# linhthi/BLISS-GNN

Measured on AMD Instinct MI355X. Metric: steps/sec (train step: sample_blocks + gather + SAGE fwd/bwd + Adam + exp3), reddit-like, higher is better.
Workload: dtype bf16

## Files before the change

### bliss_gnn_amd/csrc/sampler.hip

```cpp
#include "common.cuh"
#include "bliss_gnn.h"
#include "prof.h"
#include "edge_q.cuh"
#include <cstdlib>

#ifndef TPB
#define TPB 256
#endif
#define ITEMS 4
#define CHUNK (TPB * ITEMS)

namespace {

#define SPAN (64 * ITEMS)
#define SEG_ZERO_WGS 8
#define LONG_COL 1024
#define LONG_FIRST 4096

struct alignas(8) ColEnt {
  int k, n;
  long long p0;
};

struct EdgeAt {
// ... 522 lines not shown
        if (i < n) x[r] = wc[i];
      }
#pragma unroll
      for (int r = 0; r < COL_RB; ++r) wr.set(r, x[r]);
    }
#pragma unroll
    for (int r = 0; r < COL_RB; ++r)
      if (t + r * COL_TPB < n) emax = max(emax, bf_exp_field(wr.get(r)));
#pragma unroll 8
    for (int i = t + COL_RB * COL_TPB; i < n; i += COL_TPB) emax = max(emax, bf_exp_field(wc[i]));
    const int wfrac = rel_frac(FRAC_DST, block_max_u31<COL_TPB>(emax, sh));
    const PlainRange wr_ok = bf_plain_range(wfrac);
    bool odd = false;
#pragma unroll
    for (int r = 0; r < COL_RB; ++r)
      if (wave0 + r * COL_TPB < n) {
        odd |= t + r * COL_TPB < n && !bf_is_plain(wr.get(r), wr_ok);
        part += bf_fixed_plain(wr.get(r), wfrac);
      }
#pragma unroll 8
    for (int i = t + COL_RB * COL_TPB; i < n; i += COL_TPB) {
      const bf16_t b = wc[i];
      odd |= !bf_is_plain(b, wr_ok);
      part += bf_fixed_plain(b, wfrac);
    }
    long long lost;
    long long ws_fixed = block_sum2_i64<COL_TPB>(part, odd ? 1 : 0, sh2, &lost);
    bf16_t wsum;
    if (lost == 0) wsum = fixed_to_bf(ws_fixed, wfrac, &bad);
    else {
      long long part_lo = 0;
      int sticky = 0;
      part = 0;
#pragma unroll 4
      for (int i = t; i < n; i += COL_TPB) part += bf_to_fixed_wide(wc[i], wfrac, &part_lo, &sticky, &bad);
      ws_fixed = block_sum2_i64<COL_TPB>(part, (part_lo != 0 || sticky) ? 1 : 0, sh2, &lost);
      if (lost == 0) wsum = fixed_to_bf(ws_fixed, wfrac, &bad);
      else {
        const long long lo_tot = block_sum_i64<COL_TPB>(part_lo, sh);
        const long long st_tot = block_sum_i64<COL_TPB>(sticky, sh);
        wsum = fixed_wide_to_bf(ws_fixed, lo_tot, st_tot != 0, wfrac, &bad);
      }
    }
    const float a = rbf((1.0f / (float)n) * eta_f);
    const PlainRange q_ok = bf_plain_range(FRAC_DST);
    part = 0; odd = false;
#pragma unroll
    for (int r = 0; r < COL_RB; ++r)
      if (wave0 + r * COL_TPB < n) {
        const bool in = t + r * COL_TPB < n;
        const bf16_t q = edge_q_pre(wr.get(r), wsum, a, ome_f);
        odd |= in && !bf_is_plain(q, q_ok);
        part += in ? bf_fixed_plain(q, FRAC_DST) : 0ll;
      }
#pragma unroll 8
    for (int i = t + COL_RB * COL_TPB; i < n; i += COL_TPB) {
      const bf16_t q = edge_q_pre(wc[i], wsum, a, ome_f);
      odd |= !bf_is_plain(q, q_ok);
      part += bf_fixed_plain(q, FRAC_DST);
    }
    long long qs_fixed = block_sum2_i64<COL_TPB>(part, odd ? 1 : 0, sh2, &lost);
    if (lost != 0) {
      part = 0;
#pragma unroll 4
      for (int i = t; i < n; i += COL_TPB) part += bf_to_fixed(edge_q_pre(wc[i], wsum, a, ome_f), FRAC_DST, &bad);
      qs_fixed = block_sum_i64<COL_TPB>(part, sh);
    }
    if (t == 0) col_store(k, ws_fixed, qs_fixed, wsum, n, eta_f, acc_w, acc_q, seed_coef, &bad);
  }
  }
  if (bad) atomicOr(&cnt->err, bad);
}

template <bool BANDIT>
__global__ void __launch_bounds__(BIN_TPB) k_bin_scatter(const int64_t* __restrict__ indptr, const int* __restrict__ indices,
                                                     const bf16_t* __restrict__ w, const int* __restrict__ seeds,
                                                     const int* __restrict__ seg_ptr, const long long* __restrict__ col_base,
    const int* __restrict__ span_seg, LayerCounts* cnt,
                                                     const unsigned long long* __restrict__ acc_w,
                                                     const unsigned long long* __restrict__ acc_q, float eta_f, float ome_f,
                                                     int uniform_nodes, int n_bins, int log2_bins, long long bin_cap, int* bin_cursor,
                                                     unsigned long long* __restrict__ bin_rec, unsigned* __restrict__ bitmap,
                                                     const uint2* __restrict__ seed_coef) {
  __shared__ int hist[MAX_BINS];
  __shared__ int gbase[MAX_BINS];
  const int S = cnt->S, E = cnt->E, tid = threadIdx.x;
  const int nb = (E + BIN_BATCH - 1) / BIN_BATCH;
  const int bmask = n_bins - 1;
  int bad = 0;
  for (int batch = blockIdx.x; batch < nb; batch += gridDim.x) {
    for (int b = tid; b < n_bins; b += BIN_TPB) hist[b] = 0;
    if (tid < BIN_BATCH / 32) bitmap[batch * (BIN_BATCH / 32) + tid] = 0u;
    __syncthreads();
    int srcs[BIN_ITEMS], ranks[BIN_ITEMS];
    bf16_t ts[BIN_ITEMS];
    const int wbase = batch * BIN_BATCH + (tid >> 6) * (64 * BIN_ITEMS);
    int hint = span_seg[wbase >> 8];
#pragma unroll
    for (int j = 0; j < BIN_ITEMS; ++j) {
      ranks[j] = -1; srcs[j] = 0; ts[j] = 0;
      const int base = wbase + j * 64;
      if (base >= E) continue;
      EdgeAt a = decode(base, E, S, seg_ptr, col_base, indices, &hint);
      if (a.k >= 0) {
        bf16_t t;
        if (uniform_nodes) {
          t = (bf16_t)0x3f80;
        } else if (BANDIT) {
          const uint2 cf = seed_coef[a.k];
          bf16_t q = edge_q_pre(w[a.pos], (bf16_t)(cf.x & 0xffffu), __uint_as_float(cf.y), ome_f);
          float r = rbf(bf2f(q) / bf2f((bf16_t)(cf.x >> 16)));
          t = f2bf(r * r);
        } else {
          float x = bf2f(w[a.pos]);
          t = f2bf(x * x);
        }
        srcs[j] = a.src; ts[j] = t;
        ranks[j] = atomicAdd(&hist[a.src & bmask], 1);
      }
    }
    __syncthreads();
    for (int b = tid; b < n_bins; b += BIN_TPB) {
      const int h = hist[b];
      int g0 = 0;
      if (h) {
        g0 = atomicAdd(bin_cursor + b, h);
        if ((long long)g0 + h > bin_cap) bad |= BLISS_ERR_CAP_CAND;
      }
      gbase[b] = g0;
    }
    __syncthreads();
#pragma unroll
    for (int j = 0; j < BIN_ITEMS; ++j) {
      if (ranks[j] >= 0) {
        const int b = srcs[j] & bmask;
        const long long idx = (long long)gbase[b] + ranks[j];
        if (idx < bin_cap) {
          const size_t o = (size_t)b * (size_t)bin_cap + (size_t)idx;
          const unsigned e = (unsigned)(wbase + j * 64 + lane_id());
          bin_rec[o] = ((unsigned long long)e << 32) | ((unsigned long long)((unsigned)srcs[j] >> log2_bins) << 15) | (ts[j] & 0x7fffu);
        }
      }
    }
    __syncthreads();
  }
  if (bad) atomicOr(&cnt->err, bad);
}

__global__ void __launch_bounds__(BINRED_TPB) k_bin_reduce(LayerCounts* cnt, int n_bins, int log2_bins, long long bin_cap,
                                                           int* bin_cursor, const unsigned long long* __restrict__ bin_rec,
                                                           int num_nodes, int slots,
                                                           const int* __restrict__ local_id, unsigned long long* __restrict__ seed_p2,
                                                           unsigned long long* __restrict__ touched_key,
                                                           unsigned long long* __restrict__ touched_sum, unsigned* bitmap, int cap_c) {
  extern __shared__ unsigned long long dyn_lds[];
  unsigned long long* sm = dyn_lds;
  unsigned* mn = (unsigned*)(dyn_lds + slots);
  const int b = blockIdx.x, tid = threadIdx.x;
  if (cnt->E == 0) return;
  const int ne = b < num_nodes ? ((num_nodes - 1 - b) >> log2_bins) + 1 : 0;
  for (int i = tid; i < ne; i += BINRED_TPB) { sm[i] = 0ull; mn[i] = 0xffffffffu; }
  __syncthreads();
  long long n = bin_cursor[b];
  if (n > bin_cap) n = bin_cap;
  const unsigned long long* rec = bin_rec + (size_t)b * (size_t)bin_cap;
  int bad = 0;
  for (long long i = tid; i < n; i += BINRED_TPB) {
    const unsigned long long r = rec[i];
    const int li = (int)(((unsigned)r) >> 15);
    atomicMin(&mn[li], (unsigned)(r >> 32));
    const int64_t fx = bf_to_fixed((bf16_t)(r & 0x7fffu), FRAC_SRC, &bad);
    if (fx) atomicAdd(&sm[li], (unsigned long long)fx);
  }
  __syncthreads();
  __shared__ int wg_cnt, wg_base;
  if (tid == 0) wg_cnt = 0;
  __syncthreads();
  for (int li = tid; li < ne; li += BINRED_TPB) {
    bool is_cand = false;
    if (mn[li] != 0xffffffffu) {
      const int lid = local_id[((unsigned)li << log2_bins) | (unsigned)b];
      if (lid >= 0) { seed_p2[lid] = sm[li]; mn[li] = 0xffffffffu; }
      else is_cand = true;
    }
    const unsigned long long mask = __ballot(is_cand);
    if (mask && lane_id() == 0) atomicAdd(&wg_cnt, __popcll(mask));
  }
  __syncthreads();
  if (tid == 0) { wg_base = wg_cnt ? atomicAdd(bin_cursor + n_bins, wg_cnt) : 0; wg_cnt = 0; }
  __syncthreads();
  for (int li = tid; li < ne; li += BINRED_TPB) {
    const unsigned fp = mn[li];
    if (fp != 0xffffffffu) {
      const int j = wg_base + atomicAdd(&wg_cnt, 1);
      if (j < cap_c) { touched_key[j] = ((unsigned long long)fp << 32) | (((unsigned)li << log2_bins) | (unsigned)b); touched_sum[j] = sm[li]; }
      atomicOr(bitmap + (fp >> 5), 1u << (fp & 31u));
    }
  }
  if (bad) atomicOr(&cnt->err, bad);
}

#define BTILE_W 4
#define BTILE (1024 * BTILE_W)
#define MAX_TILES 2048
__global__ void __launch_bounds__(1024) k_bitmap_tiles(const unsigned* __restrict__ bitmap, int* __restrict__ word_prefix,
                                                       int* __restrict__ tile_sum, LayerCounts* cnt) {
  __shared__ int sh[17];
  const int nw = (cnt->E + 31) >> 5;
  const int ntiles = (nw + BTILE - 1) / BTILE;
  for (int tile = blockIdx.x; tile < ntiles; tile += gridDim.x) {
    const int i = tile * BTILE + threadIdx.x * BTILE_W;
    uint4 v = make_uint4(0, 0, 0, 0);
    if (i < nw) v = *reinterpret_cast<const uint4*>(bitmap + i);
    const int c0 = __popc(v.x), c1 = __popc(v.y), c2 = __popc(v.z), c3 = __popc(v.w);
    int total, ex = block_excl_scan(c0 + c1 + c2 + c3, sh, &total);
    if (i < nw) *reinterpret_cast<int4*>(word_prefix + i) = make_int4(ex, ex + c0, ex + c0 + c1, ex + c0 + c1 + c2);
    if (threadIdx.x == 0) tile_sum[tile] = total;
  }
}

__device__ __forceinline__ double block_sum_f64(double v, double* shd) {
  for (int d = 32; d >= 1; d >>= 1) {
    long long b = __double_as_longlong(v);
    int lo = __shfl_down((int)(b & 0xffffffffll), d), hi = __shfl_down((int)(b >> 32), d);
    v += __longlong_as_double(((long long)hi << 32) | (unsigned)lo);
  }
  __syncthreads();
  if (lane_id() == 0) shd[threadIdx.x >> 6] = v;
  __syncthreads();
  double t = 0;
  for (int i = 0; i < (int)(blockDim.x >> 6); ++i) t += shd[i];
  return t;
}

template <bool COHERENT>
__device__ __forceinline__ void poisson_scale_body(int* hist, LayerCounts* cnt, int C, int num, double eps, int* rng_ctl,
                                                   int* layer_off, int is_last, int rng_cap_total, int* __restrict__ sel_state,
                                                   double* shd) {
  for (int i = threadIdx.x; i < (C + CHUNK - 1) / CHUNK + 2; i += 1024) sel_state[i] = 0;
  if (rng_ctl && threadIdx.x == 1023) rng_stream_acquire(rng_ctl, C, layer_off, is_last, rng_cap_total);
  int n[HIST_BINS / 1024];
  bool any = false;
#pragma unroll
  for (int i = 0; i < HIST_BINS / 1024; ++i) {
    const int b = i * 1024 + threadIdx.x;
    n[i] = COHERENT ? __hip_atomic_load(hist + b, __ATOMIC_RELAXED, __HIP_MEMORY_SCOPE_AGENT) : hist[b];
  }
#pragma unroll
  for (int i = 0; i < HIST_BINS / 1024; ++i) {
    const int b = i * 1024 + threadIdx.x;
    if (n[i]) {
      if (COHERENT) __hip_atomic_store(hist + b, 0, __ATOMIC_RELAXED, __HIP_MEMORY_SCOPE_AGENT); else hist[b] = 0;
      any = true;
    }
  }
  if (C <= num) {
    if (threadIdx.x == 0) { cnt->c = 1.0; cnt->all_one = 1; cnt->iters = 0; }
    return;
  }
  double c = 1.0;
  int it = 0;
  for (; it < 50; ++it) {
    const float c32 = (float)c;
    double loc = 0;
    if (any) {
#pragma unroll
      for (int i = 0; i < HIST_BINS / 1024; ++i) {
        if (n[i]) {
          float v = rbf(bf2f((bf16_t)(i * 1024 + threadIdx.x)) * c32);
          v = v < 1.0f ? v : (v != v ? v : 1.0f);
          loc += (double)n[i] * (double)v;
        }
      }
    }
    double Ssum = block_sum_f64(loc, shd);
    double lo = Ssum < (double)num ? Ssum : (double)num, hi = Ssum < (double)num ? (double)num : Ssum;
    if (lo / hi >= eps) { ++it; break; }
    c *= (double)num / Ssum;
  }
  if (threadIdx.x == 0) { cnt->c = c; cnt->all_one = 0; cnt->iters = it > 50 ? 50 : it; }
}

__global__ void __launch_bounds__(1024) k_poisson_scale(int* hist, LayerCounts* cnt, int num, double eps, int* rng_ctl,
                                                        int* layer_off, int is_last, int rng_cap_total, int* __restrict__ sel_state) {
  __shared__ double shd[16];
  poisson_scale_body<false>(hist, cnt, cnt->C, num, eps, rng_ctl, layer_off, is_last, rng_cap_total, sel_state, shd);
}

struct FusedScale { int* ticket; int num; double eps; int* rng_ctl; int* layer_off; int is_last; int rng_cap_total; int* sel_state; };
__global__ void __launch_bounds__(FIN_TPB) k_cand_number(const int* __restrict__ seeds, LayerCounts* cnt, int* __restrict__ cand_nid,
                                                         int* local_id, const unsigned long long* __restrict__ seed_p2,
                                                         const unsigned long long* __restrict__ touched_key,
                                                         const unsigned long long* __restrict__ touched_sum,
                                                         const unsigned* __restrict__ bitmap, const int* __restrict__ word_prefix,
                                                         const int* __restrict__ tile_sum, bf16_t* __restrict__ p, int* hist,
                                                         int cap_c, int uniform_nodes, const FusedScale fs) {
  __shared__ int lh[HWIN_N + 4];
  __shared__ int tile_off[MAX_TILES];
  __shared__ int sh[17];
  const int S = cnt->S;
  const int ntiles = (((cnt->E + 31) >> 5) + BTILE - 1) / BTILE;
  int run = 0;
  for (int base = 0; base < ntiles; base += FIN_TPB) {
    const int t = base + threadIdx.x;
    int total, ex = block_excl_scan(t < ntiles ? tile_sum[t] : 0, sh, &total);
    if (t < ntiles) tile_off[t] = run + ex;
    run += total;
  }
  int C = S + run;
  if (C > cap_c) { C = cap_c; if (blockIdx.x == 0 && threadIdx.x == 0) atomicOr(&cnt->err, BLISS_ERR_CAP_CAND); }
  if (blockIdx.x == 0 && threadIdx.x == 0) cnt->C = C;
  if (blockIdx.x != 0 && (int)blockIdx.x * FIN_TPB >= C) return;
  {
    int4* lh4 = reinterpret_cast<int4*>(lh);
    for (int b = threadIdx.x; b < (HWIN_N + 4) / 4; b += FIN_TPB) lh4[b] = make_int4(0, 0, 0, 0);
  }
  __syncthreads();
  int bad = 0;
  for (int i = blockIdx.x * FIN_TPB + threadIdx.x; i < C; i += gridDim.x * FIN_TPB) {
    int id;
    unsigned long long raw;
    if (i < S) {
      id = i; raw = seed_p2[i];
      cand_nid[i] = seeds[i];
    } else {
      const unsigned long long key = touched_key[i - S];
      raw = touched_sum[i - S];
      const unsigned fp = (unsigned)(key >> 32), g = (unsigned)key;
      id = S + tile_off[(fp >> 5) / BTILE] + word_prefix[fp >> 5] + __popc(bitmap[fp >> 5] & ((1u << (fp & 31u)) - 1u));
      if (id >= cap_c) continue;
      local_id[g] = id; cand_nid[id] = (int)g;
    }
    bf16_t pj;
    if (uniform_nodes) pj = raw ? (bf16_t)0x3f80 : (bf16_t)0;
    else pj = f2bf(sqrtf(bf2f(fixed_to_bf((int64_t)raw, FRAC_SRC, &bad))));
    p[id] = pj;
    if (pj >= HIST_BINS) bad |= BLISS_ERR_NONFINITE;
    else if ((unsigned)(pj - HWIN_LO) < (unsigned)HWIN_N) atomicAdd(&lh[pj - HWIN_LO], 1);
    else if (pj == 0) atomicAdd(&lh[HWIN_N], 1);
    else atomicAdd(hist + pj, 1);
  }
  __syncthreads();
  {
    const int4* lh4 = reinterpret_cast<const int4*>(lh);
    for (int b = threadIdx.x; b < HWIN_N / 4; b += FIN_TPB) {
      const int4 v = lh4[b];
      if (v.x | v.y | v.z | v.w) {
        if (v.x) atomicAdd(hist + HWIN_LO + 4 * b, v.x);
        if (v.y) atomicAdd(hist + HWIN_LO + 4 * b + 1, v.y);
        if (v.z) atomicAdd(hist + HWIN_LO + 4 * b + 2, v.z);
        if (v.w) atomicAdd(hist + HWIN_LO + 4 * b + 3, v.w);
      }
    }
    if (threadIdx.x == 0 && lh[HWIN_N]) atomicAdd(hist, lh[HWIN_N]);
  }
  if (bad) atomicOr(&cnt->err, bad);
  if (fs.ticket) {
    static_assert(FIN_TPB == 1024, "the fused Poisson scale runs in a 1024-thread workgroup");
    __shared__ int sh_is_last;
    __shared__ double shd[16];
    int active = (C + FIN_TPB - 1) / FIN_TPB;
    if (active > (int)gridDim.x) active = (int)gridDim.x;
    if (active < 1) active = 1;
    asm volatile("s_waitcnt vmcnt(0)" ::: "memory");
    __syncthreads();
    if (threadIdx.x == 0) {
      sh_is_last = atomicAdd(fs.ticket, 1) == active - 1;
      if (sh_is_last) __hip_atomic_store(fs.ticket, 0, __ATOMIC_RELAXED, __HIP_MEMORY_SCOPE_AGENT);
    }
    __syncthreads();
    if (sh_is_last)
      poisson_scale_body<true>(hist, cnt, C, fs.num, fs.eps, fs.rng_ctl, fs.layer_off, fs.is_last, fs.rng_cap_total, fs.sel_state, shd);
  }
}

__device__ __forceinline__ bf16_t incl_prob(const bf16_t* __restrict__ p, int j, int S, int all_one, float c32) {
  if (all_one || j < S) return 0x3f80;
  float v = rbf(bf2f(p[j]) * c32);
  return (v < 1.0f || v != v) ? f2bf(v) : (bf16_t)0x3f80;
}

#define SEL_AGG 1
#define SEL_PFX 2
__global__ void __launch_bounds__(TPB) k_select_fused(const bf16_t* __restrict__ p, const float* __restrict__ uniforms_base,
                                                      const int* __restrict__ u_off, LayerCounts* cnt, bf16_t* __restrict__ P,
                                                      int* state, const int* __restrict__ cand_nid, int* __restrict__ new_id,
                                                      int* __restrict__ kept_nid, bf16_t* __restrict__ node_prob, int cap_c, int cap_k,
                                                      int* __restrict__ kept_map) {
  __shared__ int sh4[TPB / 64];
  __shared__ int sh_chunk, sh_base, sh_K;
  const float* __restrict__ uniforms = uniforms_base + (u_off ? *u_off : 0);
  const int S = cnt->S, C = min(cnt->C, cap_c), all_one = cnt->all_one;
  const float c32 = (float)cnt->c;
  const int nchunks = (C + CHUNK - 1) / CHUNK;
  if (threadIdx.x == 0) sh_chunk = atomicAdd(state, 1);
  __syncthreads();
  const int chunk = sh_chunk;
  if (chunk >= nchunks) return;
  unsigned long long mask[ITEMS];
  bf16_t Pv[ITEMS];
  int wave_total = 0;
#pragma unroll
  for (int i = 0; i < ITEMS; ++i) {
    const int j = chunk * CHUNK + (threadIdx.x >> 6) * SPAN + i * 64 + lane_id();
    bool keep = false;
    Pv[i] = 0;
    if (j < C) {
      Pv[i] = incl_prob(p, j, S, all_one, c32);
      P[j] = Pv[i];
      keep = __hip_atomic_load(uniforms + j, __ATOMIC_RELAXED, __HIP_MEMORY_SCOPE_AGENT) < bf2f(Pv[i]);
    }
    mask[i] = __ballot(keep);
    wave_total += __popcll(mask[i]);
  }
  int tot;
  const int woff = chunk_wave_offset(wave_total, sh4, &tot);
  if (threadIdx.x < 64) {
    const int lane = lane_id();
    int excl = 0, bad = 0;
    if (chunk > 0) {
      if (lane == 0) __hip_atomic_store(state + 1 + chunk, (tot << 2) | SEL_AGG, __ATOMIC_RELAXED, __HIP_MEMORY_SCOPE_AGENT);
      long long spins = 0;
      for (int top = chunk - 1; top >= 0;) {
        const int j = top - lane;
        const int v = j >= 0 ? __hip_atomic_load(state + 1 + j, __ATOMIC_RELAXED, __HIP_MEMORY_SCOPE_AGENT) : SEL_PFX;
        const unsigned long long ready = __ballot((v & 3) != 0), pfx = __ballot((v & 3) == SEL_PFX);
        const int stop = pfx ? __ffsll((long long)pfx) - 1 : 63;
        const unsigned long long need = stop == 63 ? ~0ull : ((1ull << (stop + 1)) - 1ull);
        if ((ready & need) != need) {
          __builtin_amdgcn_s_sleep(1);
          if (++spins > (1ll << 22)) { bad = BLISS_ERR_CAP_KEPT; break; }
          continue;
        }
        excl += wave_total_i32(lane <= stop && j >= 0 ? (v >> 2) : 0);
        if (pfx) break;
        top -= 64;
      }
    }
    if (lane == 0) {
      __hip_atomic_store(state + 1 + chunk, ((excl + tot) << 2) | SEL_PFX, __ATOMIC_RELAXED, __HIP_MEMORY_SCOPE_AGENT);
      sh_base = excl;
      if (chunk == nchunks - 1) {
        int K = excl + tot;
        if (K > cap_k) { bad |= BLISS_ERR_CAP_KEPT; K = cap_k; }
        cnt->K = K;
        sh_K = K;
      }
      if (bad) atomicOr(&cnt->err, bad);
    }
  }
  __syncthreads();
  int run = sh_base + woff;
#pragma unroll
  for (int i = 0; i < ITEMS; ++i) {
    const int j = chunk * CHUNK + (threadIdx.x >> 6) * SPAN + i * 64 + lane_id();
    if (j < C) {
      const bool keep = (mask[i] >> lane_id()) & 1ull;
      const int r = run + __popcll(mask[i] & ((1ull << lane_id()) - 1ull));
      if (keep && r < cap_k) {
        const int g = cand_nid[j];
        kept_nid[r] = g; node_prob[r] = Pv[i]; new_id[j] = r;
        if (kept_map) kept_map[g] = r;
      } else new_id[j] = -1;
    }
    run += __popcll(mask[i]);
  }
  if (chunk == nchunks - 1)
    for (int r = sh_K + threadIdx.x; r < cap_k; r += TPB) { kept_nid[r] = 0; node_prob[r] = 0x3f80; }
}

__global__ void __launch_bounds__(TPB) k_mn_prepare(LayerCounts* cnt, const bf16_t* __restrict__ p, bf16_t* __restrict__ P,
                                                    int* __restrict__ new_id, int cap_c) {
  const int C = min(cnt->C, cap_c);
  for (int j = blockIdx.x * TPB + threadIdx.x; j < C; j += gridDim.x * TPB) { P[j] = p[j]; new_id[j] = 0; }
}
__global__ void __launch_bounds__(TPB) k_mn_mark(LayerCounts* cnt, const int* __restrict__ chosen, int n_chosen, int* __restrict__ new_id, int cap_c) {
  const int C = min(cnt->C, cap_c);
  for (int i = blockIdx.x * TPB + threadIdx.x; i < n_chosen; i += gridDim.x * TPB) {
    const int j = chosen[i];
    if (j >= 0 && j < C) new_id[j] = 1; else atomicOr(&cnt->err, BLISS_ERR_CAP_CAND);
  }
}
__global__ void __launch_bounds__(TPB) k_mn_copy_p(const LayerCounts* cnt, const bf16_t* __restrict__ p, bf16_t* __restrict__ P, int cap_c) {
  const int C = min(cnt->C, cap_c);
  for (int j = blockIdx.x * TPB + threadIdx.x; j < C; j += gridDim.x * TPB) P[j] = p[j];
}
template <bool EMIT>
__global__ void __launch_bounds__(TPB) k_mn_select(LayerCounts* cnt, const bf16_t* __restrict__ P, int* __restrict__ chunk_io,
                                                   const int* __restrict__ cand_nid, int* __restrict__ new_id,
                                                   int* __restrict__ kept_nid, bf16_t* __restrict__ node_prob, int cap_c, int cap_k,
                                                   int* __restrict__ kept_map) {
  __shared__ int sh4[TPB / 64];
  const int S = cnt->S, C = min(cnt->C, cap_c);
  const int nchunks = (C + CHUNK - 1) / CHUNK;
  for (int chunk = blockIdx.x; chunk < nchunks; chunk += gridDim.x) {
    unsigned long long mask[ITEMS];
    int drawn[ITEMS];
    int wave_total = 0;
#pragma unroll
    for (int i = 0; i < ITEMS; ++i) {
      const int j = chunk * CHUNK + (threadIdx.x >> 6) * SPAN + i * 64 + lane_id();
      drawn[i] = j < C ? (EMIT ? new_id[j] : new_id[j] == 1) : 0;
      mask[i] = __ballot(j < C && (drawn[i] == 1 || j < S));
      wave_total += __popcll(mask[i]);
    }
    int tot;
    const int woff = chunk_wave_offset(wave_total, sh4, &tot);
    if (!EMIT) { if (threadIdx.x == 0) chunk_io[chunk] = tot; continue; }
    int run = chunk_io[chunk] + woff;
#pragma unroll
    for (int i = 0; i < ITEMS; ++i) {
      const int j = chunk * CHUNK + (threadIdx.x >> 6) * SPAN + i * 64 + lane_id();
      if (j < C) {
        const bool in_u = (mask[i] >> lane_id()) & 1ull;
        const int r = run + __popcll(mask[i] & ((1ull << lane_id()) - 1ull));
        if (in_u && r < cap_k) {
          const int g = cand_nid[j];
          kept_nid[r] = g; node_prob[r] = P[j]; new_id[j] = drawn[i] == 1 ? r : -2 - r;
          if (kept_map && drawn[i] == 1) kept_map[g] = r;
        } else new_id[j] = -1;
      }
      run += __popcll(mask[i]);
    }
  }
  if (EMIT) {
    const int K = min(cnt->K, cap_k);
// ... 200 lines not shown
}

#define TSORT_MAX_S 32768
__global__ void __launch_bounds__(TPB) k_tr_sort_lists(const int* __restrict__ t_indptr, const int* __restrict__ t_unsorted,
                                                       const int* __restrict__ dst, LayerCounts* cnt, int cap_k, int cap_s,
                                                       int* __restrict__ t_edge, const int* __restrict__ cand_nid, int* local_id,
                                                       int cap_c, const int* __restrict__ kept_nid, int* kept_map, int do_cleanup) {
  extern __shared__ unsigned bm_all[];
  if (do_cleanup) maps_cleanup(cnt, cand_nid, local_id, cap_c, kept_nid, kept_map, cap_k);
  const int lane = lane_id(), wave = threadIdx.x >> 6;
  const int words = (cap_s + 31) / 32;
  unsigned* bm = bm_all + (size_t)wave * (words + 1);
  const int K = min(cnt->K, cap_k);
  for (int j = blockIdx.x * (TPB / 64) + wave; j < K; j += gridDim.x * (TPB / 64)) {
    const int beg = t_indptr[j], len = t_indptr[j + 1] - beg;
    if (len <= 0) continue;
    if (len <= 64) {
      const int v = lane < len ? t_unsorted[beg + lane] : 0x7fffffff;
      int rank = 0;
      for (int k = 0; k < len; ++k) rank += (__shfl(v, k) < v);
      if (lane < len) t_edge[beg + rank] = v;
      continue;
    }
    for (int w = lane; w <= words; w += 64) bm[w] = 0;
    __builtin_amdgcn_fence(__ATOMIC_SEQ_CST, "wavefront"); __builtin_amdgcn_wave_barrier();
    for (int i = lane; i < len; i += 64) { const int d = dst[t_unsorted[beg + i]]; atomicOr(bm + (d >> 5), 1u << (d & 31)); }
    __builtin_amdgcn_fence(__ATOMIC_SEQ_CST, "wavefront"); __builtin_amdgcn_wave_barrier();
    int carry = 0;
    for (int base = 0; base < words; base += 64) {
      const int w = base + lane;
      const unsigned bits = w < words ? bm[w] : 0u;
      int c = __popc(bits), inc = c;
#pragma unroll
      for (int d = 1; d < 64; d <<= 1) { int t = __shfl_up(inc, d); if (lane >= d) inc += t; }
      const int excl = carry + inc - c;
      carry += __shfl(inc, 63);
      for (int i = 0; i < len; i += 64) {
        const int idx = i + lane;
        int e = 0, d = -1;
        if (idx < len) { e = t_unsorted[beg + idx]; d = dst[e]; }
        const int dw = d >> 5;
        const bool mine = idx < len && dw >= base && dw < base + 64;
        const int src_lane = mine ? dw - base : 0;
        const int ex_w = __shfl(excl, src_lane);
        const unsigned bits_w = __shfl((int)bits, src_lane);
        if (mine) t_edge[beg + ex_w + __popc(bits_w & ((1u << (d & 31)) - 1u))] = e;
      }
    }
    __builtin_amdgcn_fence(__ATOMIC_SEQ_CST, "wavefront"); __builtin_amdgcn_wave_barrier();
  }
}

__global__ void __launch_bounds__(TPB) k_cleanup(LayerCounts* cnt, const int* __restrict__ cand_nid, int* local_id, int cap_c,
                                                 const int* __restrict__ kept_nid, int* kept_map, int cap_k) {
  maps_cleanup(cnt, cand_nid, local_id, cap_c, kept_nid, kept_map, cap_k);
}

inline int grid_for(int64_t n, int per_block, int max_blocks = 8192) {
  int64_t g = (n + per_block - 1) / per_block;
  if (g < 1) g = 1;
  if (g > max_blocks) g = max_blocks;
  return (int)g;
}

}

#define CK(x) do { hipError_t e_ = (x); if (e_ != hipSuccess) return (int)e_; } while (0)

static long long g_flag_spin_bound = 1ll << 22;
__global__ void __launch_bounds__(64) k_flag_wait(int* flag, int* err, long long bound) {
  if (threadIdx.x != 0) return;
  long long spins = 0;
  while (__hip_atomic_load(flag, __ATOMIC_RELAXED, __HIP_MEMORY_SCOPE_AGENT) == 0) {
    __builtin_amdgcn_s_sleep(8);
    if (++spins > bound) { if (err) atomicOr(err, BLISS_ERR_FLAG_TIMEOUT); break; }
  }
  __builtin_amdgcn_fence(__ATOMIC_ACQUIRE, "agent");
  __hip_atomic_store(flag, 0, __ATOMIC_RELAXED, __HIP_MEMORY_SCOPE_AGENT);
}

__global__ void k_flag_raise(int* flag) {
  if (threadIdx.x == 0) __hip_atomic_store(flag, 1, __ATOMIC_RELEASE, __HIP_MEMORY_SCOPE_AGENT);
}

extern "C" {

int bliss_layer_counts_bytes(void) { return (int)sizeof(LayerCounts); }

int bliss_flag_raise(int32_t* flag, void* stream) {
  if (!flag) return BLISS_EINVAL;
  k_flag_raise<<<1, 64, 0, (hipStream_t)stream>>>(flag);
  return (int)hipGetLastError();
}

int bliss_flag_wait(int32_t* flag, int32_t* err_word, void* stream) {
  if (!flag) return BLISS_EINVAL;
  k_flag_wait<<<1, 64, 0, (hipStream_t)stream>>>(flag, err_word, g_flag_spin_bound);
  return (int)hipGetLastError();
}

int bliss_flag_set_spin_bound(int64_t spins) {
  if (spins < 1) return BLISS_EINVAL;
  g_flag_spin_bound = spins;
  return 0;
}

int bliss_frontier_prob(const bliss_graph_t* g, const bliss_node_maps_t* m, const void* w_pos, const int32_t* seeds,
                        int32_t n_seeds, const int32_t* n_seeds_dev, int32_t cap_s, int mode, float eta_f,
                        float one_minus_eta_f, int64_t frontier_bound, const bliss_layer_ws_t* ws, void* stream_) {
  if (!g || !m || !seeds || !ws || !w_pos || cap_s <= 0 || !ws->hist || !ws->span_seg) return BLISS_EINVAL;
  if (n_seeds < 0 && !n_seeds_dev) return BLISS_EINVAL;
  if (n_seeds > cap_s) return BLISS_EINVAL;
  const int uniform_nodes = (mode & BLISS_MODE_UNIFORM_NODES) ? 1 : 0;
  const bool partials_only = (mode & BLISS_MODE_PARTIALS) != 0;
  mode &= ~(BLISS_MODE_UNIFORM_NODES | BLISS_MODE_PARTIALS);
  if (mode != BLISS_MODE_BANDIT && mode != BLISS_MODE_LADIES) return BLISS_EINVAL;
  if (partials_only && ws->n_bins <= 0) return BLISS_EINVAL;
  hipStream_t st = (hipStream_t)stream_;
  LayerCounts* cnt = (LayerCounts*)ws->counts;
  const bf16_t* w = (const bf16_t*)w_pos;
  unsigned long long* acc_w = (unsigned long long*)ws->seed_acc;
  unsigned long long* acc_q = acc_w + cap_s;
  const long long* col_base = (const long long*)(acc_w + 5 * (size_t)cap_s);
  if (frontier_bound < 1) frontier_bound = 1;
  const int ge = grid_for(frontier_bound, TPB), gc = grid_for(frontier_bound, CHUNK);
  const bool binned = ws->n_bins > 0;
  int log2_bins = 0, slots = 0;
  if (binned) {
    while ((1 << log2_bins) < ws->n_bins) ++log2_bins;
    slots = (g->num_nodes + ws->n_bins - 1) >> log2_bins;
    if ((1 << log2_bins) != ws->n_bins || ws->n_bins > MAX_BINS || (size_t)slots * 12 > 64 * 1024 || ws->bin_cap <= 0 ||
        g->num_edges > (long long)MAX_TILES * BTILE * 32 || !ws->bin_cursor || !ws->bin_rec || !ws->bitmap || !ws->word_prefix || !ws->touched_key || !ws->touched_sum)
      return BLISS_EINVAL;
  }
  const long long fcap = (long long)(g->num_edges < 0x7fffffffll ? g->num_edges : 0x7fffffffll);
  const bool col_sums = binned && mode == BLISS_MODE_BANDIT;
  ColEnt* long_list = (ColEnt*)(acc_w + 7 * (size_t)cap_s);
  PROF_LAUNCH(BK_SEG_SCAN, st, k_seg_scan<<<1 + SEG_ZERO_WGS, 1024, 0, st>>>(g->indptr, seeds, cnt, n_seeds, n_seeds_dev, cap_s, acc_w, ws->seg_ptr,
                                                            m->local_id, g->num_nodes, ws->src_cnt, ws->cap_k,
                                                            binned ? ws->bin_cursor : nullptr, ws->n_bins, (long long*)col_base, ws->span_seg,
                                                            fcap, ws->entry_flag, col_sums ? 1 : 0, col_sums ? long_list : nullptr));
  if (binned) {
    unsigned long long* seed_p2 = acc_w + 4 * (size_t)cap_s;
    uint2* seed_coef = (uint2*)(acc_w + 6 * (size_t)cap_s);
    unsigned long long* bin_rec = (unsigned long long*)ws->bin_rec;
    const int gb = grid_for(frontier_bound, BIN_BATCH);
    const int n_wave_wgs = (cap_s + COL_TPB / 64 - 1) / (COL_TPB / 64), n_block_wgs = cap_s < COL_BLOCK_WGS ? cap_s : COL_BLOCK_WGS;
    if (col_sums)
      PROF_LAUNCH(BK_COL_SUMS, st, k_col_sums<<<n_block_wgs + n_wave_wgs, COL_TPB, 0, st>>>(g->indptr, w, seeds, ws->seg_ptr, col_base, ws->span_seg, cnt, acc_w, acc_q, eta_f, one_minus_eta_f, seed_coef, n_block_wgs, long_list, cap_s));
    if (mode == BLISS_MODE_BANDIT)
      PROF_LAUNCH(BK_BIN_SCATTER, st, k_bin_scatter<true><<<gb, BIN_TPB, 0, st>>>(g->indptr, g->indices, w, seeds, ws->seg_ptr, col_base, ws->span_seg, cnt, acc_w, acc_q, eta_f, one_minus_eta_f, uniform_nodes, ws->n_bins, log2_bins, ws->bin_cap, ws->bin_cursor, bin_rec, ws->bitmap, seed_coef));
    else
      PROF_LAUNCH(BK_BIN_SCATTER, st, k_bin_scatter<false><<<gb, BIN_TPB, 0, st>>>(g->indptr, g->indices, w, seeds, ws->seg_ptr, col_base, ws->span_seg, cnt, acc_w, acc_q, eta_f, one_minus_eta_f, uniform_nodes, ws->n_bins, log2_bins, ws->bin_cap, ws->bin_cursor, bin_rec, ws->bitmap, seed_coef));
    PROF_LAUNCH(BK_BIN_REDUCE, st, k_bin_reduce<<<ws->n_bins, BINRED_TPB, (size_t)slots * 12, st>>>(
        cnt, ws->n_bins, log2_bins, ws->bin_cap, ws->bin_cursor, bin_rec, g->num_nodes, slots, m->local_id, seed_p2,
        (unsigned long long*)ws->touched_key, (unsigned long long*)ws->touched_sum, ws->bitmap, ws->cap_c));
    if (partials_only) return (int)hipGetLastError();
    int* tile_sum = ws->word_prefix;
    int* word_prefix = ws->word_prefix + MAX_TILES;
    PROF_LAUNCH(BK_BITMAP_SCAN, st, k_bitmap_tiles<<<grid_for(frontier_bound, (int64_t)BTILE * 32, MAX_TILES), 1024, 0, st>>>(ws->bitmap, word_prefix, tile_sum, cnt));
    int gf = (ws->cap_c + FIN_TPB - 1) / FIN_TPB;
    if (gf < 1) gf = 1;
    if (gf > 512) gf = 512;
    PROF_LAUNCH(BK_CAND_NUMBER, st, k_cand_number<<<gf, FIN_TPB, 0, st>>>(
        seeds, cnt, ws->cand_nid, m->local_id, seed_p2, (const unsigned long long*)ws->touched_key,
        (const unsigned long long*)ws->touched_sum, ws->bitmap, word_prefix, tile_sum, (bf16_t*)ws->p, ws->hist, ws->cap_c, uniform_nodes,
        FusedScale{ws->fs_ticket, ws->fs_fanout, ws->fs_eps, ws->fs_rng_ctl, ws->fs_layer_off, ws->fs_is_last, ws->fs_rng_cap, ws->chunk_cnt}));
    return (int)hipGetLastError();
  }
  if (mode == BLISS_MODE_BANDIT) {
    PROF_LAUNCH(BK_PASS1, st, k_frontier_pass1<true><<<ge, TPB, 0, st>>>(g->indptr, g->indices, w, seeds, ws->seg_ptr, col_base, ws->span_seg, cnt, m->local_id, m->first_pos, acc_w));
    PROF_LAUNCH(BK_PASS2, st, k_frontier_pass2<true><<<gc, TPB, 0, st>>>(g->indptr, g->indices, w, seeds, ws->seg_ptr, col_base, ws->span_seg, cnt, m->first_pos, acc_w, acc_q, ws->chunk_cnt, eta_f, one_minus_eta_f));
  } else {
    PROF_LAUNCH(BK_PASS1, st, k_frontier_pass1<false><<<ge, TPB, 0, st>>>(g->indptr, g->indices, w, seeds, ws->seg_ptr, col_base, ws->span_seg, cnt, m->local_id, m->first_pos, acc_w));
    PROF_LAUNCH(BK_PASS2, st, k_frontier_pass2<false><<<gc, TPB, 0, st>>>(g->indptr, g->indices, w, seeds, ws->seg_ptr, col_base, ws->span_seg, cnt, m->first_pos, acc_w, acc_q, ws->chunk_cnt, eta_f, one_minus_eta_f));
  }
  PROF_LAUNCH(BK_CHUNK_SCAN, st, k_chunk_scan<<<1, 1024, 0, st>>>(ws->chunk_cnt, cnt, 0, ws->cap_c));
  if (mode == BLISS_MODE_BANDIT)
    PROF_LAUNCH(BK_PASS3, st, k_frontier_pass3<true><<<gc, TPB, 0, st>>>(g->indptr, g->indices, w, seeds, ws->seg_ptr, col_base, ws->span_seg, cnt, m->first_pos, acc_w, acc_q, ws->chunk_cnt, m->local_id, ws->cand_nid, (unsigned long long*)m->acc_p2, eta_f, one_minus_eta_f, ws->cap_c, uniform_nodes));
  else
    PROF_LAUNCH(BK_PASS3, st, k_frontier_pass3<false><<<gc, TPB, 0, st>>>(g->indptr, g->indices, w, seeds, ws->seg_ptr, col_base, ws->span_seg, cnt, m->first_pos, acc_w, acc_q, ws->chunk_cnt, m->local_id, ws->cand_nid, (unsigned long long*)m->acc_p2, eta_f, one_minus_eta_f, ws->cap_c, uniform_nodes));
  {
    int gf = (ws->cap_c + FIN_TPB * 8 - 1) / (FIN_TPB * 8);
    if (gf < 1) gf = 1;
    if (gf > 256) gf = 256;
    PROF_LAUNCH(BK_CAND_FINALIZE, st, k_cand_finalize<<<gf, FIN_TPB, 0, st>>>(
        seeds, cnt, ws->cand_nid, (unsigned long long*)m->acc_p2, m->first_pos, (bf16_t*)ws->p, ws->hist, ws->cap_c, uniform_nodes));
  }
  return (int)hipGetLastError();
}

int bliss_poisson_select(const bliss_layer_ws_t* ws, int32_t fanout, double eps, const float* uniforms,
                         int32_t* uniforms_offset_dev, int32_t* rng_ctl, int is_last, int32_t rng_cap_total,
                         int64_t cand_bound, void* stream_) {
  if (!ws || !uniforms || fanout < 0 || (rng_ctl && !uniforms_offset_dev)) return BLISS_EINVAL;
  hipStream_t st = (hipStream_t)stream_;
  LayerCounts* cnt = (LayerCounts*)ws->counts;
  if (cand_bound < 1) cand_bound = 1;
  if (cand_bound > ws->cap_c) cand_bound = ws->cap_c;
  if (!ws->fs_ticket)
    PROF_LAUNCH(BK_POISSON_SCALE, st, k_poisson_scale<<<1, 1024, 0, st>>>(ws->hist, cnt, fanout, eps, rng_ctl, uniforms_offset_dev, is_last, rng_cap_total, ws->chunk_cnt));
  PROF_LAUNCH(BK_SELECT2, st, k_select_fused<<<grid_for(cand_bound, CHUNK, 1 << 20), TPB, 0, st>>>(
      (const bf16_t*)ws->p, uniforms, uniforms_offset_dev, cnt, (bf16_t*)ws->P, ws->chunk_cnt, ws->cand_nid, ws->new_id, ws->kept_nid,
      (bf16_t*)ws->node_prob, ws->cap_c, ws->cap_k, ws->kept_map));
  return (int)hipGetLastError();
}

int bliss_poisson_scale(int32_t* hist, void* counts, int32_t fanout, double eps, int32_t* scratch, void* stream_) {
  if (!hist || !counts || !scratch || fanout < 0) return BLISS_EINVAL;
  hipStream_t st = (hipStream_t)stream_;
  PROF_LAUNCH(BK_POISSON_SCALE, st, k_poisson_scale<<<1, 1024, 0, st>>>(hist, (LayerCounts*)counts, fanout, eps, nullptr, nullptr, 0, 0, scratch));
  return (int)hipGetLastError();
}

int bliss_multinomial_select(const bliss_layer_ws_t* ws, const int32_t* chosen, int32_t n_chosen, void* stream_) {
  if (!ws || n_chosen < 0 || (n_chosen > 0 && !chosen)) return BLISS_EINVAL;
  hipStream_t st = (hipStream_t)stream_;
  LayerCounts* cnt = (LayerCounts*)ws->counts;
  const int gc = grid_for(ws->cap_c, CHUNK), ge = grid_for(ws->cap_c, TPB);
  k_mn_prepare<<<ge, TPB, 0, st>>>(cnt, (const bf16_t*)ws->p, (bf16_t*)ws->P, ws->new_id, ws->cap_c);
  if (n_chosen > 0) k_mn_mark<<<grid_for(n_chosen, TPB), TPB, 0, st>>>(cnt, chosen, n_chosen, ws->new_id, ws->cap_c);
  k_mn_select<false><<<gc, TPB, 0, st>>>(cnt, (const bf16_t*)ws->P, ws->chunk_cnt, ws->cand_nid, ws->new_id, ws->kept_nid, (bf16_t*)ws->node_prob, ws->cap_c, ws->cap_k, ws->kept_map);
  k_chunk_scan<<<1, 1024, 0, st>>>(ws->chunk_cnt, cnt, 1, ws->cap_k);
  k_mn_select<true><<<gc, TPB, 0, st>>>(cnt, (const bf16_t*)ws->P, ws->chunk_cnt, ws->cand_nid, ws->new_id, ws->kept_nid, (bf16_t*)ws->node_prob, ws->cap_c, ws->cap_k, ws->kept_map);
  return (int)hipGetLastError();
}

int bliss_multinomial_select_marked(const bliss_layer_ws_t* ws, void* stream_) {
  if (!ws || !ws->counts || !ws->p || !ws->P || !ws->new_id || !ws->cand_nid || !ws->chunk_cnt || !ws->kept_nid || !ws->node_prob ||
      ws->cap_c <= 0 || ws->cap_k <= 0)
    return BLISS_EINVAL;
  hipStream_t st = (hipStream_t)stream_;
  LayerCounts* cnt = (LayerCounts*)ws->counts;
  const int gc = grid_for(ws->cap_c, CHUNK), ge = grid_for(ws->cap_c, TPB);
  k_mn_copy_p<<<ge, TPB, 0, st>>>(cnt, (const bf16_t*)ws->p, (bf16_t*)ws->P, ws->cap_c);
  k_mn_select<false><<<gc, TPB, 0, st>>>(cnt, (const bf16_t*)ws->P, ws->chunk_cnt, ws->cand_nid, ws->new_id, ws->kept_nid, (bf16_t*)ws->node_prob, ws->cap_c, ws->cap_k, ws->kept_map);
  k_chunk_scan<<<1, 1024, 0, st>>>(ws->chunk_cnt, cnt, 1, ws->cap_k);
  k_mn_select<true><<<gc, TPB, 0, st>>>(cnt, (const bf16_t*)ws->P, ws->chunk_cnt, ws->cand_nid, ws->new_id, ws->kept_nid, (bf16_t*)ws->node_prob, ws->cap_c, ws->cap_k, ws->kept_map);
  return (int)hipGetLastError();
}

int bliss_build_block(const bliss_graph_t* g, const bliss_node_maps_t* m, const void* w_pos, const int32_t* seeds,
                      int32_t cap_s, int mode, float eta_f, float one_minus_eta_f, int64_t frontier_bound,
                      const bliss_layer_ws_t* ws, const bliss_block_out_t* out, void* stream_) {
  if (!g || !m || !seeds || !ws || !out || !w_pos || cap_s <= 0 || !ws->span_seg) return BLISS_EINVAL;
  mode &= ~BLISS_MODE_UNIFORM_NODES;
  if (mode != BLISS_MODE_BANDIT && mode != BLISS_MODE_LADIES) return BLISS_EINVAL;
  hipStream_t st = (hipStream_t)stream_;
  LayerCounts* cnt = (LayerCounts*)ws->counts;
  const bf16_t* w = (const bf16_t*)w_pos;
  unsigned long long* acc_w = (unsigned long long*)ws->seed_acc;
  unsigned long long* acc_wt = acc_w + 2 * (size_t)cap_s;
  int* deg_blk = (int*)(acc_w + 3 * (size_t)cap_s);
  const long long* col_base = (const long long*)(acc_w + 5 * (size_t)cap_s);
  const uint2* seed_coef = (ws->n_bins > 0 && mode == BLISS_MODE_BANDIT) ? (const uint2*)(acc_w + 6 * (size_t)cap_s) : nullptr;
  if (frontier_bound < 1) frontier_bound = 1;
  const int gc = grid_for(frontier_bound, CHUNK);
  KeptRec* kept_rec = (ws->kept_rec && ws->span_cnt && frontier_bound <= ws->kept_rec_positions) ? (KeptRec*)ws->kept_rec : nullptr;
  int* src_cnt = ws->src_cnt;
  const bool want_t = src_cnt && out->t_indptr && out->t_edge && out->t_scratch;
  if (want_t && cap_s > TSORT_MAX_S) return BLISS_EINVAL;
  int* sc = want_t ? src_cnt : nullptr;
  if (mode == BLISS_MODE_BANDIT)
    PROF_LAUNCH(BK_BLOCK1, st, k_block_pass1<true><<<gc, TPB, 0, st>>>(g->indptr, g->indices, w, seeds, ws->seg_ptr, col_base, ws->span_seg, cnt, acc_w, m->local_id, ws->new_id, (const bf16_t*)ws->P, deg_blk, acc_wt, ws->chunk_cnt, sc, eta_f, one_minus_eta_f, ws->kept_map, (const bf16_t*)ws->node_prob, seed_coef, kept_rec, ws->span_cnt, (long long)ws->kept_rec_positions));
  else
    PROF_LAUNCH(BK_BLOCK1, st, k_block_pass1<false><<<gc, TPB, 0, st>>>(g->indptr, g->indices, w, seeds, ws->seg_ptr, col_base, ws->span_seg, cnt, acc_w, m->local_id, ws->new_id, (const bf16_t*)ws->P, deg_blk, acc_wt, ws->chunk_cnt, sc, eta_f, one_minus_eta_f, ws->kept_map, (const bf16_t*)ws->node_prob, seed_coef, kept_rec, ws->span_cnt, (long long)ws->kept_rec_positions));
  PROF_LAUNCH(BK_INDPTR_SCAN, st, k_block_scans<<<want_t ? 3 : 2, 1024, 0, st>>>(ws->chunk_cnt, deg_blk, cnt, out->indptr, cap_s, out->cap_b, src_cnt, out->t_indptr, ws->cap_k));
  if (mode == BLISS_MODE_BANDIT)
    PROF_LAUNCH(BK_BLOCK2, st, k_block_pass2<true><<<gc, TPB, 0, st>>>(g->indptr, g->indices, g->eid, w, seeds, ws->seg_ptr, col_base, ws->span_seg, cnt, acc_w, m->local_id, ws->new_id, (const bf16_t*)ws->P, deg_blk, acc_wt, ws->chunk_cnt, out->src, out->dst, out->pos, out->eid, (bf16_t*)out->edge_weights, (bf16_t*)out->q_ij, sc, out->t_scratch, eta_f, one_minus_eta_f, out->cap_b, ws->kept_map, (const bf16_t*)ws->node_prob, seed_coef, kept_rec, ws->span_cnt, (long long)ws->kept_rec_positions));
  else
    PROF_LAUNCH(BK_BLOCK2, st, k_block_pass2<false><<<gc, TPB, 0, st>>>(g->indptr, g->indices, g->eid, w, seeds, ws->seg_ptr, col_base, ws->span_seg, cnt, acc_w, m->local_id, ws->new_id, (const bf16_t*)ws->P, deg_blk, acc_wt, ws->chunk_cnt, out->src, out->dst, out->pos, out->eid, (bf16_t*)out->edge_weights, (bf16_t*)out->q_ij, sc, out->t_scratch, eta_f, one_minus_eta_f, out->cap_b, ws->kept_map, (const bf16_t*)ws->node_prob, seed_coef, kept_rec, ws->span_cnt, (long long)ws->kept_rec_positions));
  if (want_t && ws->block_ready_flag) {
    PROF_LAUNCH(BK_CLEANUP, st, k_cleanup<<<grid_for(ws->cap_c, TPB), TPB, 0, st>>>(cnt, ws->cand_nid, m->local_id, ws->cap_c, ws->kept_nid, ws->kept_map, ws->cap_k));
    k_flag_raise<<<1, 64, 0, st>>>(ws->block_ready_flag);
    const size_t lds = (size_t)(TPB / 64) * ((cap_s + 31) / 32 + 1) * sizeof(unsigned);
    PROF_LAUNCH(BK_TRANSPOSE, st, k_tr_sort_lists<<<grid_for(ws->cap_k, TPB / 64), TPB, lds, st>>>(out->t_indptr, out->t_scratch, out->dst, cnt, ws->cap_k, cap_s, out->t_edge, ws->cand_nid, m->local_id, ws->cap_c, ws->kept_nid, ws->kept_map, 0));
  } else if (want_t) {
    const size_t lds = (size_t)(TPB / 64) * ((cap_s + 31) / 32 + 1) * sizeof(unsigned);
    PROF_LAUNCH(BK_TRANSPOSE, st, k_tr_sort_lists<<<grid_for(ws->cap_k, TPB / 64), TPB, lds, st>>>(out->t_indptr, out->t_scratch, out->dst, cnt, ws->cap_k, cap_s, out->t_edge, ws->cand_nid, m->local_id, ws->cap_c, ws->kept_nid, ws->kept_map, 1));
    if (ws->block_ready_flag) k_flag_raise<<<1, 64, 0, st>>>(ws->block_ready_flag);
  } else {
    PROF_LAUNCH(BK_CLEANUP, st, k_cleanup<<<grid_for(ws->cap_c, TPB), TPB, 0, st>>>(cnt, ws->cand_nid, m->local_id, ws->cap_c, ws->kept_nid, ws->kept_map, ws->cap_k));
    if (ws->block_ready_flag) k_flag_raise<<<1, 64, 0, st>>>(ws->block_ready_flag);
  }
  return (int)hipGetLastError();
}

}
```

Baseline: 1486.

## Build probability histogram in bin-reduce and run Poisson scale as extra block

```diff
diff --git a/bliss_gnn_amd/csrc/sampler.hip b/bliss_gnn_amd/csrc/sampler.hip
--- a/bliss_gnn_amd/csrc/sampler.hip
+++ b/bliss_gnn_amd/csrc/sampler.hip
@@ -698,14 +698,20 @@
                                                            int num_nodes, int slots,
                                                            const int* __restrict__ local_id, unsigned long long* __restrict__ seed_p2,
                                                            unsigned long long* __restrict__ touched_key,
-                                                           unsigned long long* __restrict__ touched_sum, unsigned* bitmap, int cap_c) {
+                                                           unsigned long long* __restrict__ touched_sum, unsigned* bitmap, int cap_c,
+                                                           int* hist, int uniform_nodes) {
   extern __shared__ unsigned long long dyn_lds[];
-  unsigned long long* sm = dyn_lds;
-  unsigned* mn = (unsigned*)(dyn_lds + slots);
+  int* lh = (int*)dyn_lds;
+  unsigned long long* sm = dyn_lds + (hist ? (HWIN_N + 4) / 2 : 0);
+  unsigned* mn = (unsigned*)(sm + slots);
   const int b = blockIdx.x, tid = threadIdx.x;
   if (cnt->E == 0) return;
   const int ne = b < num_nodes ? ((num_nodes - 1 - b) >> log2_bins) + 1 : 0;
   for (int i = tid; i < ne; i += BINRED_TPB) { sm[i] = 0ull; mn[i] = 0xffffffffu; }
+  if (hist) {
+    int4* lh4 = reinterpret_cast<int4*>(lh);
+    for (int i = tid; i < (HWIN_N + 4) / 4; i += BINRED_TPB) lh4[i] = make_int4(0, 0, 0, 0);
+  }
   __syncthreads();
   long long n = bin_cursor[b];
   if (n > bin_cap) n = bin_cap;
@@ -719,6 +725,15 @@
     if (fx) atomicAdd(&sm[li], (unsigned long long)fx);
   }
   __syncthreads();
+  auto count_p = [&](unsigned long long raw) {
+    bf16_t pj;
+    if (uniform_nodes) pj = raw ? (bf16_t)0x3f80 : (bf16_t)0;
+    else pj = f2bf(sqrtf(bf2f(fixed_to_bf((int64_t)raw, FRAC_SRC, &bad))));
+    if (pj >= HIST_BINS) bad |= BLISS_ERR_NONFINITE;
+    else if ((unsigned)(pj - HWIN_LO) < (unsigned)HWIN_N) atomicAdd(&lh[pj - HWIN_LO], 1);
+    else if (pj == 0) atomicAdd(&lh[HWIN_N], 1);
+    else atomicAdd(hist + pj, 1);
+  };
   __shared__ int wg_cnt, wg_base;
   if (tid == 0) wg_cnt = 0;
   __syncthreads();
@@ -726,8 +741,10 @@
     bool is_cand = false;
     if (mn[li] != 0xffffffffu) {
       const int lid = local_id[((unsigned)li << log2_bins) | (unsigned)b];
-      if (lid >= 0) { seed_p2[lid] = sm[li]; mn[li] = 0xffffffffu; }
-      else is_cand = true;
+      if (lid >= 0) {
+        seed_p2[lid] = sm[li]; mn[li] = 0xffffffffu;
+        if (hist) count_p(sm[li]);
+      } else is_cand = true;
     }
     const unsigned long long mask = __ballot(is_cand);
     if (mask && lane_id() == 0) atomicAdd(&wg_cnt, __popcll(mask));
@@ -741,7 +758,22 @@
       const int j = wg_base + atomicAdd(&wg_cnt, 1);
       if (j < cap_c) { touched_key[j] = ((unsigned long long)fp << 32) | (((unsigned)li << log2_bins) | (unsigned)b); touched_sum[j] = sm[li]; }
       atomicOr(bitmap + (fp >> 5), 1u << (fp & 31u));
-    }
+      if (hist) count_p(sm[li]);
+    }
+  }
+  if (hist) {
+    __syncthreads();
+    const int4* lh4 = reinterpret_cast<const int4*>(lh);
+    for (int i = tid; i < HWIN_N / 4; i += BINRED_TPB) {
+      const int4 v = lh4[i];
+      if (v.x | v.y | v.z | v.w) {
+        if (v.x) atomicAdd(hist + HWIN_LO + 4 * i, v.x);
+        if (v.y) atomicAdd(hist + HWIN_LO + 4 * i + 1, v.y);
+        if (v.z) atomicAdd(hist + HWIN_LO + 4 * i + 2, v.z);
+        if (v.w) atomicAdd(hist + HWIN_LO + 4 * i + 3, v.w);
+      }
+    }
+    if (tid == 0 && lh[HWIN_N]) atomicAdd(hist, lh[HWIN_N]);
   }
   if (bad) atomicOr(&cnt->err, bad);
 }
@@ -779,7 +811,7 @@
   return t;
 }
 
-template <bool COHERENT>
+template <bool ADD_MISSING>
 __device__ __forceinline__ void poisson_scale_body(int* hist, LayerCounts* cnt, int C, int num, double eps, int* rng_ctl,
                                                    int* layer_off, int is_last, int rng_cap_total, int* __restrict__ sel_state,
                                                    double* shd) {
@@ -790,19 +822,26 @@
 #pragma unroll
   for (int i = 0; i < HIST_BINS / 1024; ++i) {
     const int b = i * 1024 + threadIdx.x;
-    n[i] = COHERENT ? __hip_atomic_load(hist + b, __ATOMIC_RELAXED, __HIP_MEMORY_SCOPE_AGENT) : hist[b];
+    n[i] = hist[b];
   }
 #pragma unroll
   for (int i = 0; i < HIST_BINS / 1024; ++i) {
     const int b = i * 1024 + threadIdx.x;
     if (n[i]) {
-      if (COHERENT) __hip_atomic_store(hist + b, 0, __ATOMIC_RELAXED, __HIP_MEMORY_SCOPE_AGENT); else hist[b] = 0;
+      hist[b] = 0;
       any = true;
     }
   }
   if (C <= num) {
     if (threadIdx.x == 0) { cnt->c = 1.0; cnt->all_one = 1; cnt->iters = 0; }
     return;
+  }
+  if (ADD_MISSING) {
+    int seen = 0;
+#pragma unroll
+    for (int i = 0; i < HIST_BINS / 1024; ++i) seen += n[i];
+    const int missing = C - (int)block_sum_f64((double)seen, shd);
+    if (threadIdx.x == 0 && missing > 0) { n[0] += missing; any = true; }
   }
   double c = 1.0;
   int it = 0;
@@ -828,9 +867,11 @@
 }
 
 __global__ void __launch_bounds__(1024) k_poisson_scale(int* hist, LayerCounts* cnt, int num, double eps, int* rng_ctl,
-                                                        int* layer_off, int is_last, int rng_cap_total, int* __restrict__ sel_state) {
+                                                        int* layer_off, int is_last, int rng_cap_total, int* __restrict__ sel_state,
+                                                        int add_missing) {
   __shared__ double shd[16];
-  poisson_scale_body<false>(hist, cnt, cnt->C, num, eps, rng_ctl, layer_off, is_last, rng_cap_total, sel_state, shd);
+  if (add_missing) poisson_scale_body<true>(hist, cnt, cnt->C, num, eps, rng_ctl, layer_off, is_last, rng_cap_total, sel_state, shd);
+  else poisson_scale_body<false>(hist, cnt, cnt->C, num, eps, rng_ctl, layer_off, is_last, rng_cap_total, sel_state, shd);
 }
 
 struct FusedScale { int* ticket; int num; double eps; int* rng_ctl; int* layer_off; int is_last; int rng_cap_total; int* sel_state; };
@@ -840,11 +881,20 @@
                                                          const unsigned long long* __restrict__ touched_sum,
                                                          const unsigned* __restrict__ bitmap, const int* __restrict__ word_prefix,
                                                          const int* __restrict__ tile_sum, bf16_t* __restrict__ p, int* hist,
-                                                         int cap_c, int uniform_nodes, const FusedScale fs) {
-  __shared__ int lh[HWIN_N + 4];
+                                                         int cap_c, int uniform_nodes, const int* __restrict__ new_cands,
+                                                         const FusedScale fs) {
   __shared__ int tile_off[MAX_TILES];
   __shared__ int sh[17];
   const int S = cnt->S;
+  if (fs.ticket && blockIdx.x == 0) {
+    static_assert(FIN_TPB == 1024, "the fused Poisson scale runs in a 1024-thread workgroup");
+    __shared__ double shd[16];
+    const long long Cs = (long long)S + *new_cands;
+    poisson_scale_body<true>(hist, cnt, Cs < cap_c ? (int)Cs : cap_c, fs.num, fs.eps, fs.rng_ctl, fs.layer_off, fs.is_last,
+                             fs.rng_cap_total, fs.sel_state, shd);
+    return;
+  }
+  const int blk = (int)blockIdx.x - (fs.ticket ? 1 : 0), nblk = (int)gridDim.x - (fs.ticket ? 1 : 0);
   const int ntiles = (((cnt->E + 31) >> 5) + BTILE - 1) / BTILE;
   int run = 0;
   for (int base = 0; base < ntiles; base += FIN_TPB) {
@@ -854,16 +904,12 @@
     run += total;
   }
   int C = S + run;
-  if (C > cap_c) { C = cap_c; if (blockIdx.x == 0 && threadIdx.x == 0) atomicOr(&cnt->err, BLISS_ERR_CAP_CAND); }
-  if (blockIdx.x == 0 && threadIdx.x == 0) cnt->C = C;
-  if (blockIdx.x != 0 && (int)blockIdx.x * FIN_TPB >= C) return;
-  {
-    int4* lh4 = reinterpret_cast<int4*>(lh);
-    for (int b = threadIdx.x; b < (HWIN_N + 4) / 4; b += FIN_TPB) lh4[b] = make_int4(0, 0, 0, 0);
-  }
+  if (C > cap_c) { C = cap_c; if (blk == 0 && threadIdx.x == 0) atomicOr(&cnt->err, BLISS_ERR_CAP_CAND); }
+  if (blk == 0 && threadIdx.x == 0) cnt->C = C;
+  if (blk != 0 && blk * FIN_TPB >= C) return;
   __syncthreads();
   int bad = 0;
-  for (int i = blockIdx.x * FIN_TPB + threadIdx.x; i < C; i += gridDim.x * FIN_TPB) {
+  for (int i = blk * FIN_TPB + threadIdx.x; i < C; i += nblk * FIN_TPB) {
     int id;
     unsigned long long raw;
     if (i < S) {
@@ -882,42 +928,8 @@
     else pj = f2bf(sqrtf(bf2f(fixed_to_bf((int64_t)raw, FRAC_SRC, &bad))));
     p[id] = pj;
     if (pj >= HIST_BINS) bad |= BLISS_ERR_NONFINITE;
-    else if ((unsigned)(pj - HWIN_LO) < (unsigned)HWIN_N) atomicAdd(&lh[pj - HWIN_LO], 1);
-    else if (pj == 0) atomicAdd(&lh[HWIN_N], 1);
-    else atomicAdd(hist + pj, 1);
-  }
-  __syncthreads();
-  {
-    const int4* lh4 = reinterpret_cast<const int4*>(lh);
-    for (int b = threadIdx.x; b < HWIN_N / 4; b += FIN_TPB) {
-      const int4 v = lh4[b];
-      if (v.x | v.y | v.z | v.w) {
-        if (v.x) atomicAdd(hist + HWIN_LO + 4 * b, v.x);
-        if (v.y) atomicAdd(hist + HWIN_LO + 4 * b + 1, v.y);
-        if (v.z) atomicAdd(hist + HWIN_LO + 4 * b + 2, v.z);
-        if (v.w) atomicAdd(hist + HWIN_LO + 4 * b + 3, v.w);
-      }
-    }
-    if (threadIdx.x == 0 && lh[HWIN_N]) atomicAdd(hist, lh[HWIN_N]);
   }
   if (bad) atomicOr(&cnt->err, bad);
-  if (fs.ticket) {
-    static_assert(FIN_TPB == 1024, "the fused Poisson scale runs in a 1024-thread workgroup");
-    __shared__ int sh_is_last;
-    __shared__ double shd[16];
-    int active = (C + FIN_TPB - 1) / FIN_TPB;
-    if (active > (int)gridDim.x) active = (int)gridDim.x;
-    if (active < 1) active = 1;
-    asm volatile("s_waitcnt vmcnt(0)" ::: "memory");
-    __syncthreads();
-    if (threadIdx.x == 0) {
-      sh_is_last = atomicAdd(fs.ticket, 1) == active - 1;
-      if (sh_is_last) __hip_atomic_store(fs.ticket, 0, __ATOMIC_RELAXED, __HIP_MEMORY_SCOPE_AGENT);
-    }
-    __syncthreads();
-    if (sh_is_last)
-      poisson_scale_body<true>(hist, cnt, C, fs.num, fs.eps, fs.rng_ctl, fs.layer_off, fs.is_last, fs.rng_cap_total, fs.sel_state, shd);
-  }
 }
 
 __device__ __forceinline__ bf16_t incl_prob(const bf16_t* __restrict__ p, int j, int S, int all_one, float c32) {
@@ -1424,9 +1436,16 @@
       PROF_LAUNCH(BK_BIN_SCATTER, st, k_bin_scatter<true><<<gb, BIN_TPB, 0, st>>>(g->indptr, g->indices, w, seeds, ws->seg_ptr, col_base, ws->span_seg, cnt, acc_w, acc_q, eta_f, one_minus_eta_f, uniform_nodes, ws->n_bins, log2_bins, ws->bin_cap, ws->bin_cursor, bin_rec, ws->bitmap, seed_coef));
     else
       PROF_LAUNCH(BK_BIN_SCATTER, st, k_bin_scatter<false><<<gb, BIN_TPB, 0, st>>>(g->indptr, g->indices, w, seeds, ws->seg_ptr, col_base, ws->span_seg, cnt, acc_w, acc_q, eta_f, one_minus_eta_f, uniform_nodes, ws->n_bins, log2_bins, ws->bin_cap, ws->bin_cursor, bin_rec, ws->bitmap, seed_coef));
-    PROF_LAUNCH(BK_BIN_REDUCE, st, k_bin_reduce<<<ws->n_bins, BINRED_TPB, (size_t)slots * 12, st>>>(
+    const size_t red_lds = (size_t)slots * 12 + (partials_only ? 0 : (size_t)(HWIN_N + 4) * sizeof(int));
+    static size_t red_lds_set = 64 * 1024;
+    if (red_lds > red_lds_set) {
+      if (hipFuncSetAttribute((const void*)k_bin_reduce, hipFuncAttributeMaxDynamicSharedMemorySize, (int)red_lds) != hipSuccess) return BLISS_EINVAL;
+      red_lds_set = red_lds;
+    }
+    PROF_LAUNCH(BK_BIN_REDUCE, st, k_bin_reduce<<<ws->n_bins, BINRED_TPB, red_lds, st>>>(
         cnt, ws->n_bins, log2_bins, ws->bin_cap, ws->bin_cursor, bin_rec, g->num_nodes, slots, m->local_id, seed_p2,
-        (unsigned long long*)ws->touched_key, (unsigned long long*)ws->touched_sum, ws->bitmap, ws->cap_c));
+        (unsigned long long*)ws->touched_key, (unsigned long long*)ws->touched_sum, ws->bitmap, ws->cap_c,
+        partials_only ? nullptr : ws->hist, uniform_nodes));
     if (partials_only) return (int)hipGetLastError();
     int* tile_sum = ws->word_prefix;
     int* word_prefix = ws->word_prefix + MAX_TILES;
@@ -1434,10 +1453,11 @@
     int gf = (ws->cap_c + FIN_TPB - 1) / FIN_TPB;
     if (gf < 1) gf = 1;
     if (gf > 512) gf = 512;
+    if (ws->fs_ticket) ++gf;
     PROF_LAUNCH(BK_CAND_NUMBER, st, k_cand_number<<<gf, FIN_TPB, 0, st>>>(
         seeds, cnt, ws->cand_nid, m->local_id, seed_p2, (const unsigned long long*)ws->touched_key,
         (const unsigned long long*)ws->touched_sum, ws->bitmap, word_prefix, tile_sum, (bf16_t*)ws->p, ws->hist, ws->cap_c, uniform_nodes,
-        FusedScale{ws->fs_ticket, ws->fs_fanout, ws->fs_eps, ws->fs_rng_ctl, ws->fs_layer_off, ws->fs_is_last, ws->fs_rng_cap, ws->chunk_cnt}));
+        ws->bin_cursor + ws->n_bins, FusedScale{ws->fs_ticket, ws->fs_fanout, ws->fs_eps, ws->fs_rng_ctl, ws->fs_layer_off, ws->fs_is_last, ws->fs_rng_cap, ws->chunk_cnt}));
     return (int)hipGetLastError();
   }
   if (mode == BLISS_MODE_BANDIT) {
@@ -1471,7 +1491,8 @@
   if (cand_bound < 1) cand_bound = 1;
   if (cand_bound > ws->cap_c) cand_bound = ws->cap_c;
   if (!ws->fs_ticket)
-    PROF_LAUNCH(BK_POISSON_SCALE, st, k_poisson_scale<<<1, 1024, 0, st>>>(ws->hist, cnt, fanout, eps, rng_ctl, uniforms_offset_dev, is_last, rng_cap_total, ws->chunk_cnt));
+    PROF_LAUNCH(BK_POISSON_SCALE, st, k_poisson_scale<<<1, 1024, 0, st>>>(ws->hist, cnt, fanout, eps, rng_ctl, uniforms_offset_dev, is_last, rng_cap_total, ws->chunk_cnt,
+                                                                          ws->n_bins > 0 ? 1 : 0));
   PROF_LAUNCH(BK_SELECT2, st, k_select_fused<<<grid_for(cand_bound, CHUNK, 1 << 20), TPB, 0, st>>>(
       (const bf16_t*)ws->p, uniforms, uniforms_offset_dev, cnt, (bf16_t*)ws->P, ws->chunk_cnt, ws->cand_nid, ws->new_id, ws->kept_nid,
       (bf16_t*)ws->node_prob, ws->cap_c, ws->cap_k, ws->kept_map));
@@ -1481,7 +1502,7 @@
 int bliss_poisson_scale(int32_t* hist, void* counts, int32_t fanout, double eps, int32_t* scratch, void* stream_) {
   if (!hist || !counts || !scratch || fanout < 0) return BLISS_EINVAL;
   hipStream_t st = (hipStream_t)stream_;
-  PROF_LAUNCH(BK_POISSON_SCALE, st, k_poisson_scale<<<1, 1024, 0, st>>>(hist, (LayerCounts*)counts, fanout, eps, nullptr, nullptr, 0, 0, scratch));
+  PROF_LAUNCH(BK_POISSON_SCALE, st, k_poisson_scale<<<1, 1024, 0, st>>>(hist, (LayerCounts*)counts, fanout, eps, nullptr, nullptr, 0, 0, scratch, 0));
   return (int)hipGetLastError();
 }
 
```

Result: no change. 1479 (-0.5%).
